# roncapat/UNIGE-TASI-path-planners

Hardware: AMD Instinct MI355X
Metric: grid cells updated/sec (full plan + 100 replans), 4096^2 map (higher is better)
Workload: dtype f32

## Files before the change

unige-tasi-path-planners_amd/csrc/ufm_control.h:

```cpp
#pragma once

__global__ void k_fill(float *p, size_t n, float v) {
    for (size_t i = (size_t)blockIdx.x * blockDim.x + threadIdx.x; i < n; i += (size_t)gridDim.x * blockDim.x) p[i] = v;
}

__device__ __forceinline__ void patch_apply(const DevParams &P, int m, const uint8_t *patch, uint8_t *pmask, int x, int y, int w, int h, int e) {
    if (e >= w * h) return;
    const int i = e / w, j = e - i * w;
    uint8_t *cm = P.cost + (size_t)m * P.cstride;
    const size_t ci = (size_t)(x + i) * P.W + (y + j);
    const uint8_t nv = patch[e];
    const uint8_t ch = cm[ci] != nv;
    pmask[e] = ch;
    if (ch) { cm[ci] = nv; cost_window_store(P, m, x + i, y + j, nv); }
}
__global__ void k_patch_apply(DevParams P, int m, const uint8_t *patch, uint8_t *pmask, int x, int y, int w, int h) {
    patch_apply(P, m, patch, pmask, x, y, w, h, blockIdx.x * blockDim.x + threadIdx.x);
}
template <bool NODES>
__device__ __forceinline__ void patch_seed(const DevParams &P, int m, const uint8_t *pmask, int x, int y, int w, int h, int e) {
    const int ew = NODES ? w + 1 : w, eh = NODES ? h + 1 : h;
    bool hit = false;
    int gt = -1;
    if (e < ew * eh) {
// ... 305 lines not shown
            else if (ug - ur > 8) ++n_low;
            else {
                const int miss = dep_dfm(ga, gp, th) & ~(b & 3);
                auto moved = [&](float v) { return v == INFINITY || abs(__float_as_int(v) - ur) > 8; };
                if (((miss & 1) && moved(q_dfm(INFINITY, gp, th))) || ((miss & 2) && moved(q_dfm(ga, INFINITY, th)))) {
                    if (below_key()) ++n_dep; else ++n_parked;
                }
            }
            continue;
        }
        const int cx = x - 1 + (q >> 1), cy = y - 1 + (q & 1);
        const float c = cst(cx, cy), g1 = h ? val(x, y + dy) : val(x + dx, y), g2 = val(x + dx, y + dy);
        float r; int dep;
        if constexpr (ALGO == UFM_ALGO_SG) { CellSG k; k.set(c); r = tri_sg(g1, g2, k); dep = dep_sg(g1, g2, k); }
        else {
            const float bb = h ? cst(x - 1 + (1 - (q >> 1)), cy) : cst(cx, y - 1 + (1 - (q & 1)));
            CellFD k{c, c * c, c * SQRT2F}; TriFD t; t.set(c, bb);
            r = tri_fd(g1, g2, k, t); dep = dep_fd(g1, g2, k, t);
        }
        if (r > g || r != r) {
            const float B = P.dyn->focused ? start_bound(P, m) : INFINITY;
            if (g + tile_heuristic(P, m, x / T, y / T) < B || B == INFINITY) ++n_bad; else ++n_parked;
        }
        else if (r < g) ++n_low;
        else if (dep != (b & 3)) ++n_dep;
    }
    if (n_val) atomicAdd(&out[0], n_val);
    if (n_none) atomicAdd(&out[1], n_none);
    if (n_bad) atomicAdd(&out[2], n_bad);
    if (n_dep) atomicAdd(&out[3], n_dep);
    if (n_low) atomicAdd(&out[4], n_low);
    if (n_parked) atomicAdd(&out[5], n_parked);
}
__global__ void k_cost_stats(const uint8_t *cm, size_t n, int thr, unsigned long long *out) {
    unsigned long long s = 0, c = 0;
    for (size_t i = (size_t)blockIdx.x * blockDim.x + threadIdx.x; i < n; i += (size_t)gridDim.x * blockDim.x) {
        const int v = cm[i];
        if (v < thr) { s += v; ++c; }
    }
    for (int o = 32; o > 0; o >>= 1) { s += __shfl_down(s, o); c += __shfl_down(c, o); }
    if ((threadIdx.x & 63) == 0) { atomicAdd(&out[0], s); atomicAdd(&out[1], c); }
}
__device__ __forceinline__ void finalize_tiles(const DevParams &P) {
    const int n = P.ctr->tcount;
    for (int i = blockIdx.x; i < n; i += gridDim.x) {
        const int gt = P.tlist[i];
        const size_t gidx = (size_t)gt * TT + threadIdx.x;
        const int diff = (threadIdx.x < T * T) && (P.fresh[gt] ? (P.G[gidx] != INFINITY) : (P.G[gidx] != P.Gprev[gidx]));
        const int c = __syncthreads_count(diff);
        if (threadIdx.x == 0) {
            if (c) atomicAdd(&P.ctr->expanded, (unsigned long long)c);
            P.touched[gt] = 0;
        }
    }
}
__global__ __launch_bounds__(256) void k_finalize(DevParams P, int only_if_done) {
    if (only_if_done && !P.ctr->done) return;
    const int n = P.ctr->tcount;
    const int lane = threadIdx.x & 63;
    const int wave = (blockIdx.x * blockDim.x + threadIdx.x) >> 6, nwaves = (gridDim.x * blockDim.x) >> 6;
    unsigned long long total = 0;
    for (int i = wave; i < n; i += nwaves) {
        const int gt = P.tlist[i];
        const float *g = P.G + (size_t)gt * TT, *g0 = P.Gprev + (size_t)gt * TT;
        int c = 0;
        if (P.fresh[gt]) {
#pragma unroll
            for (int e = lane; e < TT; e += 64) c += (g[e] != INFINITY) ? 1 : 0;
        } else {
#pragma unroll
            for (int e = lane; e < TT; e += 64) c += (g[e] != g0[e]) ? 1 : 0;
        }
        total += (unsigned long long)c;
        if (lane == 0) P.touched[gt] = 0;
    }
    for (int o = 32; o > 0; o >>= 1) total += __shfl_down(total, o);
    if (lane == 0 && total) atomicAdd(&P.ctr->expanded, total);
}
template <int ALGO>
__device__ void tile_bp(const DevParams &P, int gt, int thr, float *Gs, float *Cs) {
    constexpr int CROWS = is_dfm<ALGO> ? T : T + 1, COFF = is_dfm<ALGO> ? 0 : 1, CN = CROWS * CROWS;
    const int tid = threadIdx.x, w = tid >> 6, lane = tid & 63, q = lane & 3, nd = lane >> 2;
    const int m = gt / P.NTm, t = gt - m * P.NTm, tx = t / P.TY, ty = t - tx * P.TY, x0 = tx * T, y0 = ty * T;
    const float *Gt = P.G + (size_t)gt * TT, *ring = P.ring + (size_t)gt * RING;
    const uint8_t *ct = P.costT + (size_t)gt * CTS;
    for (int e = tid; e < TT; e += 256) Gs[(e / T + 1) * GP + e % T + 1] = Gt[e];
    for (int ht = tid; ht < 4 * T + 4; ht += 256) {
        int hr, hc;
        if (ht < T) { hr = -1; hc = ht; }
        else if (ht < 2 * T) { hr = T; hc = ht - T; }
        else if (ht < 3 * T) { hr = ht - 2 * T; hc = -1; }
        else if (ht < 4 * T) { hr = ht - 3 * T; hc = T; }
        else { hr = (ht & 2) ? T : -1; hc = (ht & 1) ? T : -1; }
        Gs[(hr + 1) * GP + hc + 1] = ring[ht];
    }
    for (int e = tid; e < CN; e += 256) {
        const int cr = e / CROWS, cc = e - cr * CROWS, cx = x0 + cr - COFF, cy = y0 + cc - COFF, c = ct[e];
        Cs[cr * CP + cc] = (cx < 0 || cy < 0 || cx >= P.L || cy >= P.W || c >= thr) ? INFINITY : (float)c;
    }
    __syncthreads();
    const int goal_x = P.goal[2 * m], goal_y = P.goal[2 * m + 1];
    for (int p = w; p < PT * PT; p += 4) {
        const int lx = (p / PT) * 4 + (nd >> 2), ly = (p % PT) * 4 + (nd & 3);
        QuadConsts<ALGO> C;
        C.load(Cs, lx, ly, q);
        const LaneEval le = eval_quad_w<ALGO>(Gs + (lx + 1) * GP + ly + 1, q, C);
        const float nv = quad_min(le.r);
        const int bq = quad_min_int(bp_byte<ALGO>(le, q, C, le.r == nv)), b = bp_of_key<ALGO>(bq);
        if (q == 0) P.bp[(size_t)gt * TT + lx * T + ly] = (uint8_t)((x0 + lx == goal_x && y0 + ly == goal_y) ? BP_NONE : b);
    }
    __syncthreads();
}
template <int ALGO>
__global__ __launch_bounds__(256) void k_finalize_bp(DevParams P, int only_if_done) {
    __shared__ float Gs[(T + 2) * GP];
    __shared__ float Cs[(T + 1) * CP];
    if (only_if_done && !P.ctr->done) return;
    const int n = P.ctr->tcount, thr = P.dyn->thr;
    for (int i = blockIdx.x; i < n; i += gridDim.x) tile_bp<ALGO>(P, P.tlist[i], thr, Gs, Cs);
}
__global__ __launch_bounds__(T * T) void k_replan_end(DevParams P, int kr, int kl, float margin,
                                                      DevCounters *host, unsigned int *flag, unsigned int seq) {
    __shared__ int s_m, s_done, s_last;
    kr = launch_index(P, Q_RAISE, kr);
    kl = launch_index(P, Q_LOWER, kl);
    if (seq == 0) seq = P.ctr->pubseq;
    const int done = replan_check(P, kr, kl, margin, blockIdx.x == 0, s_m, s_done);
    if (done) finalize_tiles(P);
    __threadfence();
    __syncthreads();
    if (threadIdx.x == 0) s_last = (atomicAdd(&P.ctr->fin_blocks, 1) == (int)gridDim.x - 1);
    __syncthreads();
    if (!s_last) return;
    __threadfence();
    if (threadIdx.x == 0) P.ctr->fin_blocks = 0;
    const int *src = reinterpret_cast<const int *>(P.ctr);
    int *dst = reinterpret_cast<int *>(host);
    for (int i = threadIdx.x; i < (int)(sizeof(DevCounters) / sizeof(int)); i += blockDim.x)
        dst[i] = __hip_atomic_load(&src[i], __ATOMIC_RELAXED, __HIP_MEMORY_SCOPE_AGENT);
    __threadfence_system();
    __syncthreads();
    if (threadIdx.x == 0) __hip_atomic_store(flag, seq, __ATOMIC_RELEASE, __HIP_MEMORY_SCOPE_SYSTEM);
}
struct ReplanBegin { StepBegin sb; int nrect; int rect[4][5]; int k_raise; float band; };
__device__ void replan_begin(const DevParams &P, const ReplanBegin &a, int &s_keep) {
    step_begin(P, a.sb);
    for (int r = 0; r < a.nrect; ++r) {
        const int *q = a.rect[r];
        for (int e = threadIdx.x; e < (q[3] + 1) * (q[4] + 1); e += blockDim.x) clear_mark(P, q[0], q[1], q[2], q[3], q[4], e);
    }
    __syncthreads();
    seeds_to_active(P, Q_RAISE, a.k_raise, s_keep);
// ... 31 lines not shown
```

unige-tasi-path-planners_amd/csrc/ufm_engine.hip:

```cpp
#include <hip/hip_runtime.h>
#include <hip/hip_ext.h>

#include <algorithm>
#include <chrono>
#include <climits>
#include <cmath>
#include <cstddef>
#include <cstdint>
#include <cstdio>
#include <cstdlib>
#include <cstring>
#include <memory>
#include <new>
#include <type_traits>
#include <thread>
#include <vector>

#include "../../include/ufm.h"

namespace {

#include "ufm_defs.h"
#include "ufm_ops.h"
#include "ufm_relax.h"
#include "ufm_control.h"

#include "ufm_region.h"
#include "ufm_cspace.h"
#include "ufm_census.h"
#include "ufm_sensor.h"
#include "ufm_prepare.h"
#include "ufm_layers.h"

#include "ufm_host.h"
#include "ufm_map_host.h"
#include "ufm_delta.h"

}

struct ufm_planner { Engine *e; };
struct ufm_batch { std::vector<Engine *> shards; int n_maps = 0, per = 1; };

extern "C" {

#ifdef UFM_SWEEPSTAT
int ufm_debug_sstat(unsigned long long *out, int reset) {
    if (out && hipMemcpyFromSymbol(out, HIP_SYMBOL(g_sstat), sizeof(unsigned long long) * 32) != hipSuccess) return UFM_ERR_HIP_BASE;
    if (reset) { unsigned long long z[32] = {}; if (hipMemcpyToSymbol(HIP_SYMBOL(g_sstat), z, sizeof(z)) != hipSuccess) return UFM_ERR_HIP_BASE; }
    return UFM_OK;
}
#endif
#ifdef UFM_TIMING
int ufm_debug_trace(unsigned long long *out, int cap) {
    unsigned int n = 0;
    if (hipMemcpyFromSymbol(&n, HIP_SYMBOL(g_ntrace), sizeof(n)) != hipSuccess) return UFM_ERR_HIP_BASE;
    if ((int)n > cap) n = cap;
    if (n > 16384) n = 16384;
    if (n && hipMemcpyFromSymbol(out, HIP_SYMBOL(g_trace), sizeof(unsigned long long) * 4 * n) != hipSuccess) return UFM_ERR_HIP_BASE;
    const unsigned int z = 0;
    hipMemcpyToSymbol(HIP_SYMBOL(g_ntrace), &z, sizeof(z));
// ... 503 lines not shown
```

unige-tasi-path-planners_amd/csrc/ufm_host.h:

```cpp
#pragma once

#define HIPCHK(expr)                                                      \
    do {                                                                  \
        hipError_t _e = (expr);                                           \
        if (_e != hipSuccess) return UFM_ERR_HIP_BASE - (int)_e;          \
    } while (0)

#include "ufm_route.h"
#include "ufm_patch_route.h"
#include "ufm_path.h"

static_assert(RJOBS <= ROUTE_MAX_JOBS && RTMAX >= 3, "ufm_route.h places at most ROUTE_MAX_JOBS blocks");
constexpr RouteConfig ROUTE_CONFIG{T, RTMAX, RJOBS, ROUTE_MAX_RECTS, 65 * 65};

template <int V> using IntC = std::integral_constant<int, V>;
template <class F> void with_lower_op(int algo, F &&f) {
    if (algo == UFM_ALGO_FD) f(IntC<UFM_ALGO_FD>{});
    else if (algo == UFM_ALGO_SG) f(IntC<UFM_ALGO_SG>{});
    else f(IntC<ALGO_DFM1>{});
}
template <class F> void with_raise_op(int algo, bool follow_info, F &&f) {
    if (algo == UFM_ALGO_DFM && follow_info) f(IntC<ALGO_DFM1_INFO>{});
    else with_lower_op(algo, f);
}
// ... 58 lines not shown
    bool fuse_control = true;
    bool use_graph = true;
    bool use_owned = true;
    float owned_limit_ms = -1.0f;
    float owned_band = -1.0f;
    uint32_t owned_launches = 0;
    EventSet<2> own_ev;
    EventSet<2> reg_ev;
    bool own_timed = false;
    int owned_flags = 0;
    int owned_waves = 0;
    bool dfm_follow_info = false;
    bool use_region = true;
    int region_ahead = 2;
    int region_tiles = 6;
    int region_sweeps = 4096;
    int region_debug = 0;
    float region_band = 1.5f;
    uint32_t region_runs = 0, region_done = 0;
    uint32_t region_cont = 0, region_cont_done = 0;
    int cont_raise = 4, cont_lower = 8;
    int batch_margin = 1;
    float raise_margin = 0.25f;
    PinArray<ReplanJob> h_job;
    struct GraphSig { DevParams P; float band, delta; int max_iters, grid, follow; };
    GraphSig graph_sig{};
    std::vector<std::pair<int, hipGraphExec_t>> graphs;
    void relax(int mode, bool dyn, dim3 g, int k_arg, float delta, float rbound, hipEvent_t e0 = nullptr, hipEvent_t e1 = nullptr);
    float band_delta(float scale) const { return delta_abs >= 0.0f ? delta_abs : scale * T * mean_cost; }
    void finalize_bp(int only_if_done) {
        if (algo == UFM_ALGO_DFM && opt_lvl < 1) return;
        with_lower_op(algo, [&](auto a) { k_finalize_bp<a()><<<2048, 256, 0, stream>>>(P, only_if_done); });
    }
    int tail_grid = 96;
    int replan_graph(int nr, int nl, float band, hipGraphExec_t *out);
    void drop_graphs() { for (auto &g : graphs) hipGraphExecDestroy(g.second); graphs.clear(); }
    struct StepScratch {
        PinArray<unsigned long long> acc;
        int *consume = nullptr, *init = nullptr, *init_tiles = nullptr;
        int *goals = nullptr;
        unsigned int *num_updated = nullptr;
        int *start_el = nullptr;
        float *start_pos = nullptr;
        int carve(int n) {
            { int rc = acc.alloc(2 + 6 * (size_t)n); if (rc != UFM_OK) return rc; }
            consume = reinterpret_cast<int *>(acc + 2); init = consume + n; init_tiles = init + n; goals = init_tiles + n;
            num_updated = reinterpret_cast<unsigned int *>(goals + 2 * n); start_el = goals + 3 * n;
            start_pos = reinterpret_cast<float *>(start_el + 4 * n);
            return UFM_OK;
        }
    } scratch;
    int *d_scratch = nullptr;
    GrowArray<float> d_field;
    GrowArray<int32_t> d_info;
    GrowArray<PathJob> d_jobs;
    GrowArray<float> d_path;
    std::vector<MapState> maps;
    std::vector<PatchRect> pending;
    int iter[2] = {0, 0};
    bool focused = true;
    bool start_cell_floor = false;
    bool dynamic_mode = true;
    PinArray<float> h_bnd;
    int last_active = 1;
    int grid_relax = 512;
    int dyn_grid = 256;
    int small_grid = 1 << 30;
    int max_iters = 32;
    float delta_abs = -1.0f;
    float delta_scale = 1.5f;
    float delta_scale_long = 2.0f;
    float mean_cost = 1.0f;
    int batch_fixed = 0;
    bool profiling = false;
    EventSet<4> chain_ev;
    std::vector<EventSet<1>> batch_ev;
    int batch_ev_slot = 64;
    hipEvent_t batch_event(int slot, int i) const { return batch_ev[(size_t)slot * batch_ev_slot + i][0]; }
    ufm_stats last{};

    std::vector<DevRow> buffer_rows();
    int alloc(int width, int length);
    void release();
    void launch_relax(int mode, float rbound, hipEvent_t e0 = nullptr, hipEvent_t e1 = nullptr);
    int fetch_counters();
    int wait_published();
    int wait_flag(const unsigned int *flag, unsigned int seq);
    int win_raise[6] = {8, 8, 8, 8, 8, 8}, win_lower[6] = {8, 8, 8, 8, 8, 8}, win_pos = 0;
    int run_phase(int mode, float rbound, uint32_t *launches, float *kernel_ms, uint32_t *timed);
    int owned_phase();
    void own_layout(int ys) {
        P.own_ys = ys; P.own_nw = 16 << ys;
        P.own_sx = (P.TX + 15) / 16; P.own_sy = (P.TY + (1 << ys) - 1) >> ys;
        P.own_slots = nmaps * P.own_sx * P.own_sy;
    }
    size_t own_words() const {
        const size_t sx = (size_t)(P.TX + 15) / 16;
        return (size_t)nmaps * sx * std::max<size_t>(256 * (size_t)((P.TY + 15) / 16), 512 * (size_t)((P.TY + 31) / 32));
    }
    int profile_stride = 4;
    int reset_queues();
    int read_bounds(float *bmax);
    struct StepRun {
        StepPlan plan;
        ufm_stats st;
// ... 718 lines not shown
        uint32_t ll = 0;
        k_unpark<<<1, 1024, 0, stream>>>(P, Q_LOWER, iter[Q_LOWER], INFINITY);
        int owned_left = -1;
        if (use_owned && pl.n_init > 0 && round == 0 && dyn_grid >= 256) {
            int rc = owned_phase();
            if (rc != UFM_OK) return rc;
            st.launches += 1u;
            st.resident_launches += 1u;
            rc = fetch_counters();
            if (rc != UFM_OK) return rc;
            owned_left = h_ctr->cnt[Q_LOWER][iter[Q_LOWER] % 3];
        }
        int rc = owned_left == 0 ? UFM_OK : run_phase(MODE_LOWER, INFINITY, &ll, &st.kernel_ms, &st.timed_launches);
        if (rc != UFM_OK) return rc;
        st.launches += ll;
        bool again = false;
        if (focused && do_raise) {
            float bnew = 0.0f;
            rc = read_bounds(&bnew);
            if (rc != UFM_OK) return rc;
            k_queue_min<<<1, 1024, 0, stream>>>(P, Q_RAISE, iter[Q_RAISE]);
            rc = fetch_counters();
            if (rc != UFM_OK) return rc;
            float qm;
            std::memcpy(&qm, &h_ctr->qmin[Q_RAISE], sizeof(float));
            if (qm < bnew) { again = true; rbound = std::fmax(bnew, rbound) + r.band; }
        }
        const auto tc = std::chrono::steady_clock::now();
        r.u_acc += std::chrono::duration<double, std::milli>(tb - ta).count();
        r.p_acc += std::chrono::duration<double, std::milli>(tc - tb).count();
        if (!again) break;
    }
    const auto td = std::chrono::steady_clock::now();
    finalize_bp(0);
    k_finalize<<<2048, 256, 0, stream>>>(P, 0);
    { int rc = fetch_counters(); if (rc != UFM_OK) return rc; }
    copy_counters(st);
    if (st.resident_launches) {
        st.resident_tile_visits = h_ctr->own_vis1 - h_ctr->own_vis0;
        st.resident_stops = (uint32_t)h_ctr->own_stops;
        if (own_timed) HIPCHK(hipEventElapsedTime(&st.resident_kernel_ms, own_ev[0], own_ev[1]));
    }
    if (profiling) {
        std::vector<int> lm(LMAX);
        HIPCHK(hipMemcpy(lm.data(), P.lmax, sizeof(int) * LMAX, hipMemcpyDeviceToHost));
        for (int v : lm) st.crit_sweeps += (uint64_t)v;
    }
    r.p_acc += std::chrono::duration<double, std::milli>(std::chrono::steady_clock::now() - td).count();
    return UFM_OK;
}

void Engine::copy_counters(ufm_stats &st) const {
    st.expanded = h_ctr->expanded;
    st.tile_visits = h_ctr->tile_visits;
    st.tile_iters = h_ctr->tile_iters;
    st.elem_evals = h_ctr->elem_evals;
    st.raise_tile_visits = h_ctr->raise_visits;
}

int Engine::step(ufm_stats *out, const float *auto_mult) {
    for (int m = 0; m < nmaps; ++m) if (!maps[m].have_map) return UFM_LOOP_FAILURE_NO_GRAPH;
    for (int m = 0; m < nmaps; ++m) if (!maps[m].goal_set) return UFM_LOOP_FAILURE_NO_GOAL;
    StepRun r{};
    r.t0 = std::chrono::steady_clock::now();
    r.nr = r.nl = 1;
    for (int i = 0; i < 6; ++i) { r.nr = std::max(r.nr, win_raise[i] + batch_margin); r.nl = std::max(r.nl, win_lower[i] + batch_margin); }
    r.plan = plan_step(ROUTE_CONFIG, route_switches(), maps.data(), pending.data(), (int)pending.size(), (int)lazy.size(), r.nr, r.nl,
                       scratch.consume, scratch.init);
    const StepPlan &pl = r.plan;
    float mult = heuristic_multiplier;
    if (auto_multiplier && heur) {
        if (auto_mult) mult = *auto_mult;
        else { int mn = 0, mx = 0; const int rc = census_minmax(&mn, &mx); if (rc != UFM_OK) return rc; mult = (float)mn; }
    }
    last_multiplier = mult;
    r.dyn_now = DevDyn{heur ? mult : 0.0f, thr_uchar, focused ? 1 : 0, 0};
    r.dyn_pending = std::memcmp(&r.dyn_now, &dyn_dev, sizeof(DevDyn)) != 0;
    r.band = raise_margin * band_delta(delta_scale);
    { int rc = begin_step(r); if (rc != UFM_OK) return rc; }
    r.t_seed = std::chrono::steady_clock::now();
    if (pl.route == Route::SeedsOnly) { int rc = seed_only(r); if (rc != UFM_OK) return rc; }
    else if (pl.route != Route::None) { int rc = replan(r); if (rc != UFM_OK) return rc; }
    if (r.n_init_tiles > 0) {
        HIPCHK(hipMemcpyAsync(d_scratch, scratch.init_tiles, sizeof(int) * r.n_init_tiles, hipMemcpyHostToDevice, stream));
        k_activate_list<<<1, 64, 0, stream>>>(P, Q_LOWER, iter[Q_LOWER], d_scratch, r.n_init_tiles);
    }
    const bool do_plan = (pl.n_init > 0 || r.updated > 0 || (pl.have_seeds && pl.n_upd > 0)) && !r.fast_done;
    r.u_acc = std::chrono::duration<double, std::milli>(std::chrono::steady_clock::now() - r.t0).count();
    if (do_plan) {
        int rc = converge(r);
        if (rc != UFM_OK) return rc;
    } else if (r.fast_done) {
        copy_counters(r.st);
        const double dt = std::chrono::duration<double, std::milli>(std::chrono::steady_clock::now() - r.t_seed).count();
        r.u_acc += 0.5 * dt;
        r.p_acc += 0.5 * dt;
    } else {
        HIPCHK(hipStreamSynchronize(stream));
    }
    for (int m = 0; m < nmaps; ++m) maps[m].new_goal = maps[m].initialize_search = false;
    ufm_stats &st = r.st;
    st.updated = r.updated;
    st.queued_lower = (uint32_t)(h_ctr->cnt[Q_LOWER][iter[Q_LOWER] % 3] + h_ctr->npark[Q_LOWER]);
    st.queued_raise = (uint32_t)(h_ctr->cnt[Q_RAISE][iter[Q_RAISE] % 3] + h_ctr->npark[Q_RAISE]);
    st.graphs_instantiated = graphs_made;
    st.region_replans = region_runs; st.region_replans_done = region_done;
    reveal_busy = false;
    st.u_ms = (float)r.u_acc;
    st.p_ms = (float)r.p_acc;
    last = st;
    if (out) *out = st;
    return UFM_OK;
}

int engine_create(Engine **out, int n_maps, int algo, int opt_lvl, int use_heuristic, int device_id) {
    if (!out || n_maps < 1 || algo < 0 || algo > 2 || opt_lvl < 0 || opt_lvl > 2) return UFM_ERR_INVALID;
    if (algo != UFM_ALGO_SG && opt_lvl > 1) return UFM_ERR_INVALID;
    int ndev = 0;
    HIPCHK(hipGetDeviceCount(&ndev));
    if (device_id < 0 || device_id >= ndev) return UFM_ERR_INVALID;
    HIPCHK(hipSetDevice(device_id));
    std::unique_ptr<Engine> e(new (std::nothrow) Engine());
    if (!e) return UFM_ERR_NOMEM;
    e->algo = algo; e->opt_lvl = opt_lvl; e->heur = use_heuristic; e->device = device_id; e->nmaps = n_maps;
    if (algo == UFM_ALGO_DFM && n_maps == 1) { e->delta_scale = e->delta_scale_long = 2.5f; e->max_iters = 16; }
    if (algo == UFM_ALGO_DFM) { e->cont_lower = 0; e->region_tiles = 8; e->region_ahead = 3; }
    e->maps.resize(n_maps);
    hipDeviceProp_t prop;
    HIPCHK(hipGetDeviceProperties(&prop, device_id));
    e->grid_relax = prop.multiProcessorCount * 2;
    e->dyn_grid = prop.multiProcessorCount;
    HIPCHK(hipStreamCreateWithFlags(&e->stream.s, hipStreamNonBlocking));
    for (Published<DevCounters> *pub : {&e->h_ctr, &e->h_pipe_ctr[0], &e->h_pipe_ctr[1]}) { int rc = pub->alloc(); if (rc != UFM_OK) return rc; }
    { int rc = e->h_job.alloc(1, Pin::Coherent); if (rc != UFM_OK) return rc; }
    std::memset(e->h_job, 0, sizeof(ReplanJob));
    {
        hipGraph_t g = nullptr;
        hipGraphExec_t ge = nullptr;
        if (hipStreamBeginCapture(e->stream, hipStreamCaptureModeThreadLocal) == hipSuccess) {
            k_fill<<<1, 64, 0, e->stream>>>(reinterpret_cast<float *>(e->h_job.p), 0, 0.0f);
            if (hipStreamEndCapture(e->stream, &g) == hipSuccess && g) {
                if (hipGraphInstantiate(&ge, g, nullptr, nullptr, 0) == hipSuccess && ge) {
                    (void)hipGraphLaunch(ge, e->stream);
                    (void)hipStreamSynchronize(e->stream);
                    (void)hipGraphExecDestroy(ge);
                }
                (void)hipGraphDestroy(g);
            }
        }
        (void)hipGetLastError();
    }
    { int rc = e->scratch.carve(n_maps); if (rc != UFM_OK) return rc; }
    { int rc = e->h_bnd.alloc(n_maps); if (rc != UFM_OK) return rc; }
    *out = e.release();
    return UFM_OK;
}

int engine_destroy(Engine *e) {
    if (!e) return UFM_ERR_INVALID;
    delete e;
    return UFM_OK;
}

int engine_set_goal(Engine *e, int m, float x, float y) {
    if (!e || m < 0 || m >= e->nmaps) return UFM_ERR_INVALID;
    MapState &ms = e->maps[m];
    const int ex = (int)std::roundf(x), ey = (int)std::roundf(y);
    ms.new_goal = !ms.goal_set ? true : (ex != ms.goal_ex || ey != ms.goal_ey);
// ... 167 lines not shown
```

unige-tasi-path-planners_amd/csrc/ufm_map_host.h:

```cpp
#pragma once

constexpr PatchRouteConfig PATCH_ROUTE_CONFIG{PATCH_MULTI, 4096, 64, Engine::LAZY_SLOTS};

int Engine::flush_deferred() {
    { int rc = flush_lazy(); if (rc != UFM_OK) return rc; }
    return flush_deferred_only();
}
int Engine::flush_deferred_only() {
    if (deferred.empty()) return UFM_OK;
    PatchMulti a{};
    a.n = (int)deferred.size();
    for (int i = 0; i < a.n; ++i) {
        const DeferredPatch &d = deferred[i];
        put_rect(a.rect[i], PatchRect{d.m, d.x, d.y, d.w, d.h});
        a.ptr[i] = d.ptr;
    }
    deferred.clear();
    with_elements(algo, [&](auto nodes) { k_patch_multi<nodes()><<<a.n, 1024, 0, stream>>>(P, a, d_pmask.dev); });
    HIPCHK(hipGetLastError());
    return UFM_OK;
}
int Engine::ensure_pmask(size_t need) {
    if (need <= d_pmask.cap) return UFM_OK;
    { int rc = flush_deferred_only(); if (rc != UFM_OK) return rc; }
// ... 292 lines not shown
        for (int k = 0; k < n_layers; ++k) j.survey[k] = d_lsurvey[k];
        j.cstride = P.cstride; j.lstride = lstride; j.slot_stride = stride;
        j.n = n_layers; j.nmaps = nmaps; j.L = L; j.W = W; j.mh = sensor.mh; j.mw = sensor.mw; j.ar = sensor.ar; j.ac = sensor.ac;
        hipEvent_t e0, e1;
        { int rc = layer_events(&e0, &e1); if (rc != UFM_OK) return rc; }
        launch(k_reveal_layers, grid, block, stream, e0, e1, j);
    } else {
        RevealJob j{};
        j.mask = d_sensor; j.survey = d_lsurvey[0]; j.cur = cs.on ? d_raw : P.cost; j.slots = d_reveal.dev; j.count = d_reveal_cnt; j.centres = h_centres;
        j.cstride = P.cstride; j.slot_stride = stride;
        j.L = L; j.W = W; j.mh = sensor.mh; j.mw = sensor.mw; j.ar = sensor.ar; j.ac = sensor.ac;
        launch(k_reveal, grid, block, stream, nullptr, nullptr, j);
    }
    HIPCHK(hipGetLastError());
    reveal_busy = true;
    for (int m = first; m < nmaps; ++m) {
        if (centres[2 * m] < 0) continue;
        const int rc = route_patch(PatchSource::RevealSlot, false, 0, d_reveal.dev + stride * (size_t)m, slot_rect(m));
        if (rc != UFM_OK) return rc;
    }
    return UFM_OK;
}
int Engine::reveal_counts(const int32_t *centres, uint64_t *changed) {
    std::vector<unsigned int> cnt((size_t)nmaps, 0u);
    bool any = false;
    for (int m = 0; m < nmaps; ++m) any = any || centres[2 * m] >= 0;
    if (any) HIPCHK(hipMemcpyAsync(cnt.data(), d_reveal_cnt, sizeof(unsigned int) * nmaps, hipMemcpyDeviceToHost, stream));
    HIPCHK(hipStreamSynchronize(stream));
    reveal_busy = false;
    for (int m = 0; m < nmaps; ++m) changed[m] = centres[2 * m] >= 0 ? cnt[m] : 0u;
    return UFM_OK;
}

template <class Fill> int engine_new_raster(Engine *e, int m, int width, int length, Fill &&fill) {
    HIPCHK(hipSetDevice(e->device));
    if (e->allocated) { int rc = e->flush_deferred(); if (rc != UFM_OK) return rc; }
    if (!e->allocated || width != e->W || length != e->L) {
        bool others = false;
        for (int k = 0; k < e->nmaps; ++k) if (k != m && e->maps[k].have_map) others = true;
        if (e->allocated && others) return UFM_ERR_INVALID;
        int rc = e->alloc(width, length);
        if (rc != UFM_OK) return rc;
        if (e->census_on) HIPCHK(hipMemsetAsync(e->d_census, 0, sizeof(uint32_t) * CENSUS_BINS * e->nmaps, e->stream));
    }
    { int rc = fill((e->cs.on ? e->d_raw : e->P.cost) + (size_t)m * e->P.cstride); if (rc != UFM_OK) return rc; }
    if (e->n_layers > 1) {
        HIPCHK(hipMemcpyAsync(e->layer_ptr(0, m), (e->cs.on ? e->d_raw : e->P.cost) + (size_t)m * e->P.cstride, e->P.cstride, hipMemcpyDeviceToDevice, e->stream));
        for (int k = 1; k < e->n_layers; ++k) HIPCHK(hipMemsetAsync(e->layer_ptr(k, m), 0, e->P.cstride, e->stream));
    }
    if (e->cs.on) e->cspace_dilate(m, e->P.cost + (size_t)m * e->P.cstride, width, PatchRect{m, 0, 0, width, length});
    if (e->census_on) { e->census_build(m); e->census_publish(); }
    k_cost_windows<<<2048, 256, 0, e->stream>>>(e->P, m);
    {
        unsigned long long *d_acc = reinterpret_cast<unsigned long long *>(e->d_scratch);
        HIPCHK(hipMemsetAsync(d_acc, 0, 2 * sizeof(unsigned long long), e->stream));
        k_cost_stats<<<512, 256, 0, e->stream>>>(e->P.cost + (size_t)m * e->P.cstride, (size_t)width * length, e->thr_uchar, d_acc);
        unsigned long long *h_acc = e->scratch.acc;
        HIPCHK(hipMemcpyAsync(h_acc, d_acc, 2 * sizeof(unsigned long long), hipMemcpyDeviceToHost, e->stream));
        HIPCHK(hipStreamSynchronize(e->stream));
        if (h_acc[1] > 0) e->mean_cost = (float)((double)h_acc[0] / (double)h_acc[1]);
    }
    if (e->track) { int rc = e->track_reset(m); if (rc != UFM_OK) return rc; }
    e->maps[m].have_map = true;
    MapState &ms = e->maps[m];
    if (ms.goal_set) ms.goal_elem_valid = ms.goal_ex >= 0 && ms.goal_ey >= 0 && ms.goal_ex < e->P.EX && ms.goal_ey < e->P.EY;
    return UFM_OK;
}

int engine_set_map(Engine *e, int m, const uint8_t *src, bool on_device, int width, int length) {
    if (!e || !src || m < 0 || m >= e->nmaps || width <= 0 || length <= 0) return UFM_ERR_INVALID;
    return engine_new_raster(e, m, width, length, [&](uint8_t *dst) -> int {
        HIPCHK(hipMemcpyAsync(dst, src, (size_t)width * length, on_device ? hipMemcpyDeviceToDevice : hipMemcpyHostToDevice, e->stream));
        return UFM_OK;
    });
}

int engine_set_image(Engine *e, int m, const uint8_t *src, bool on_device, int width, int length, const uint16_t *taps, int ntaps, int penalty) {
    PrepTaps k;
    if (!e || !src || m < 0 || m >= e->nmaps || !prep_args_valid(taps, ntaps, width, length, penalty) || !prep_pack(taps, ntaps, &k)) return UFM_ERR_INVALID;
    if (e->allocated && (width != e->W || length != e->L))
        for (int j = 0; j < e->nmaps; ++j) if (j != m && e->maps[j].have_map) return UFM_ERR_INVALID;
    bool timed = false;
    const int rc = engine_new_raster(e, m, width, length, [&](uint8_t *dst) -> int {
        const size_t n = (size_t)width * length, all = e->P.cstride * e->nmaps;
        { int rc2 = e->survey_alloc(0); if (rc2 != UFM_OK) return rc2; }
        uint8_t *survey = e->d_lsurvey[0];
        const uint8_t *image = src;
        if (!on_device || prep_overlap(src, n, e->P.cost, all) || prep_overlap(src, n, survey, all) || (e->cs.on && prep_overlap(src, n, e->d_raw, all))) {
            { int rc2 = e->d_image.reserve(e->stream, n); if (rc2 != UFM_OK) return rc2; }
            HIPCHK(hipMemcpyAsync(e->d_image.dev, src, n, on_device ? hipMemcpyDeviceToDevice : hipMemcpyHostToDevice, e->stream));
            image = e->d_image.dev;
        }
        PrepareJob j{};
        j.src = image; j.out_l = dst; j.out_h = survey + (size_t)m * e->P.cstride;
        j.W = width; j.L = length; j.penalty = penalty;
        j.wide_in = width % 4 == 0 && prep_aligned4(j.src);
        j.wide_out = width % 4 == 0 && prep_aligned4(j.out_l) && prep_aligned4(j.out_h);
        j.taps = k;
        timed = e->profiling;
        if (timed) { int rc2 = e->prep_ev.ensure(); if (rc2 != UFM_OK) return rc2; }
        launch(k_prepare, dim3(prep_grid_x(width), prep_grid_y(length)), dim3(PREP_THREADS), e->stream, timed ? e->prep_ev[0] : nullptr,
               timed ? e->prep_ev[1] : nullptr, j);
        HIPCHK(hipGetLastError());
        e->have_lsurvey[0][m] = 1;
        return UFM_OK;
    });
    if (rc != UFM_OK) return rc;
    e->reveal_busy = false;
    if (timed) HIPCHK(hipEventElapsedTime(&e->prep_ms, e->prep_ev[0], e->prep_ev[1]));
    return UFM_OK;
}

int engine_read_map(Engine *e, int m, uint8_t *host_map) {
    if (!e || !host_map || !e->allocated || m < 0 || m >= e->nmaps) return UFM_ERR_INVALID;
    HIPCHK(hipSetDevice(e->device));
    { int rc = e->flush_deferred(); if (rc != UFM_OK) return rc; }
// ... 12 lines not shown
```

unige-tasi-path-planners_amd/csrc/ufm_ops.h:

```cpp
#pragma once

#ifdef UFM_SWEEPSTAT
__device__ unsigned long long g_sstat[32];
#endif
__device__ __forceinline__ float sqrt_rn(float x) {
    float s = __builtin_amdgcn_sqrtf(x);
    const float sm = __int_as_float(__float_as_int(s) - 1);
    const float sp = __int_as_float(__float_as_int(s) + 1);
    const float rm = __builtin_fmaf(-sm, s, x);
    const float rp = __builtin_fmaf(-sp, s, x);
    s = (rm <= 0.0f) ? sm : s;
    s = (rp > 0.0f) ? sp : s;
    return s;
}

struct CellSG {
    float cadd;
    float ccmp;
    float c2, cs2;
    __device__ __forceinline__ void set(float c) {
        cadd = c; ccmp = (c == INFINITY) ? -1.0f : c; c2 = c * c; cs2 = c * SQRT2F;
    }
};
__device__ __forceinline__ float tri_sg(float g1, float g2, const CellSG &K) {
// ... 176 lines not shown
}
template <int ALGO, int GPITCH = GP>
__device__ __forceinline__ float eval_quad(const float *ctr, int q, const QuadConsts<ALGO> &C) {
    if constexpr (ALGO == ALGO_DFM1) {
        const float pm = fminf(ctr[-C.po], ctr[C.po]);
        return fminf(q_dfm(ctr[-C.so], pm, C.th), q_dfm(ctr[C.so], pm, C.th));
    } else {
        const int sx = (q & 2) ? GPITCH : -GPITCH, sy = (q & 1) ? 1 : -1;
        const float gD = ctr[sx + sy], gV = ctr[sx], gH = ctr[sy];
        if constexpr (ALGO == UFM_ALGO_SG)
            return fminf(tri_sg(gV, gD, C.k), tri_sg(gH, gD, C.k));
        else
            return fminf(tri_fd(gV, gD, C.k, C.tv), tri_fd(gH, gD, C.k, C.th));
    }
}

__device__ __forceinline__ void cost_window_store(const DevParams &P, int m, int cx, int cy, uint8_t v) {
    const int bx = cx / T, by = cy / T, rx = cx % T, ry = cy % T;
    if (P.cells) {
        P.costT[((size_t)m * P.NTm + (size_t)bx * P.TY + by) * CTS + rx * T + ry] = v;
        return;
    }
#pragma unroll
    for (int dx = 0; dx < 2; ++dx)
#pragma unroll
        for (int dy = 0; dy < 2; ++dy) {
            if ((dx && rx != T - 1) || (dy && ry != T - 1)) continue;
            const int tx = bx + dx, ty = by + dy;
            if (tx >= P.TX || ty >= P.TY) continue;
            const int cr = dx ? 0 : rx + 1, cc = dy ? 0 : ry + 1;
            P.costT[((size_t)m * P.NTm + (size_t)tx * P.TY + ty) * CTS + cr * (T + 1) + cc] = v;
        }
}
__global__ void k_cost_windows(DevParams P, int m) {
    const int crows = P.cells ? T : T + 1, off = P.cells ? 0 : 1, per = crows * crows;
    const uint8_t *cm = P.cost + (size_t)m * P.cstride;
    const size_t n = (size_t)P.NTm * per;
    for (size_t i = (size_t)blockIdx.x * blockDim.x + threadIdx.x; i < n; i += (size_t)gridDim.x * blockDim.x) {
        const int t = (int)(i / per), e = (int)(i - (size_t)t * per);
        const int tx = t / P.TY, ty = t - tx * P.TY, cr = e / crows, cc = e - cr * crows;
        const int cx = tx * T + cr - off, cy = ty * T + cc - off;
        const bool in = cx >= 0 && cy >= 0 && cx < P.L && cy < P.W;
        P.costT[((size_t)m * P.NTm + t) * CTS + e] = in ? cm[(size_t)cx * P.W + cy] : (uint8_t)255;
    }
}
```

Measured before the change: 598.9 million.

## Fuse cost window build with cost stats and defer mean-cost sync; fuse finalize count into bp

Replaces the separate cost-window kernel and cost-stats reduction with one tile-per-wave kernel. It reads each map row with wide loads, writes the tile window through LDS, and accumulates the mean-cost sums in the same pass. The host synchronize after map upload is deferred until the mean cost is actually needed at the next step, using a flag published by the last block. Full-plan finalization now counts changed cells inside the backpointer kernel instead of launching a second finalize kernel. The cost is more complex last-block reduction and flag logic, plus a risk of stale mean_cost ordering.

```diff
diff --git a/unige-tasi-path-planners_amd/csrc/ufm_control.h b/unige-tasi-path-planners_amd/csrc/ufm_control.h
--- a/unige-tasi-path-planners_amd/csrc/ufm_control.h
+++ b/unige-tasi-path-planners_amd/csrc/ufm_control.h
@@ -361,15 +361,6 @@
     if (n_low) atomicAdd(&out[4], n_low);
     if (n_parked) atomicAdd(&out[5], n_parked);
 }
-__global__ void k_cost_stats(const uint8_t *cm, size_t n, int thr, unsigned long long *out) {
-    unsigned long long s = 0, c = 0;
-    for (size_t i = (size_t)blockIdx.x * blockDim.x + threadIdx.x; i < n; i += (size_t)gridDim.x * blockDim.x) {
-        const int v = cm[i];
-        if (v < thr) { s += v; ++c; }
-    }
-    for (int o = 32; o > 0; o >>= 1) { s += __shfl_down(s, o); c += __shfl_down(c, o); }
-    if ((threadIdx.x & 63) == 0) { atomicAdd(&out[0], s); atomicAdd(&out[1], c); }
-}
 __device__ __forceinline__ void finalize_tiles(const DevParams &P) {
     const int n = P.ctr->tcount;
     for (int i = blockIdx.x; i < n; i += gridDim.x) {
@@ -406,13 +397,22 @@
     for (int o = 32; o > 0; o >>= 1) total += __shfl_down(total, o);
     if (lane == 0 && total) atomicAdd(&P.ctr->expanded, total);
 }
-template <int ALGO>
-__device__ void tile_bp(const DevParams &P, int gt, int thr, float *Gs, float *Cs) {
+template <int ALGO, bool COUNT = false>
+__device__ int tile_bp(const DevParams &P, int gt, int thr, float *Gs, float *Cs) {
     constexpr int CROWS = is_dfm<ALGO> ? T : T + 1, COFF = is_dfm<ALGO> ? 0 : 1, CN = CROWS * CROWS;
     const int tid = threadIdx.x, w = tid >> 6, lane = tid & 63, q = lane & 3, nd = lane >> 2;
     const int m = gt / P.NTm, t = gt - m * P.NTm, tx = t / P.TY, ty = t - tx * P.TY, x0 = tx * T, y0 = ty * T;
     const float *Gt = P.G + (size_t)gt * TT, *ring = P.ring + (size_t)gt * RING;
     const uint8_t *ct = P.costT + (size_t)gt * CTS;
+    int changed = 0;
+    if constexpr (COUNT) {
+        const float *G0 = P.fresh[gt] ? nullptr : P.Gprev + (size_t)gt * TT;
+        for (int e = tid; e < TT; e += 256) {
+            const float g = Gt[e];
+            Gs[(e / T + 1) * GP + e % T + 1] = g;
+            changed += (G0 ? g != G0[e] : g != INFINITY) ? 1 : 0;
+        }
+    } else
     for (int e = tid; e < TT; e += 256) Gs[(e / T + 1) * GP + e % T + 1] = Gt[e];
     for (int ht = tid; ht < 4 * T + 4; ht += 256) {
         int hr, hc;
@@ -439,6 +439,7 @@
         if (q == 0) P.bp[(size_t)gt * TT + lx * T + ly] = (uint8_t)((x0 + lx == goal_x && y0 + ly == goal_y) ? BP_NONE : b);
     }
     __syncthreads();
+    return changed;
 }
 template <int ALGO>
 __global__ __launch_bounds__(256) void k_finalize_bp(DevParams P, int only_if_done) {
@@ -447,6 +448,26 @@
     if (only_if_done && !P.ctr->done) return;
     const int n = P.ctr->tcount, thr = P.dyn->thr;
     for (int i = blockIdx.x; i < n; i += gridDim.x) tile_bp<ALGO>(P, P.tlist[i], thr, Gs, Cs);
+}
+template <int ALGO>
+__global__ __launch_bounds__(256) void k_finalize_count_bp(DevParams P) {
+    __shared__ float Gs[(T + 2) * GP];
+    __shared__ float Cs[(T + 1) * CP];
+    __shared__ unsigned long long s_cnt[4];
+    const int n = P.ctr->tcount, thr = P.dyn->thr;
+    unsigned long long total = 0;
+    for (int i = blockIdx.x; i < n; i += gridDim.x) {
+        const int gt = P.tlist[i];
+        total += (unsigned long long)tile_bp<ALGO, true>(P, gt, thr, Gs, Cs);
+        if (threadIdx.x == 0) P.touched[gt] = 0;
+    }
+    for (int o = 32; o > 0; o >>= 1) total += __shfl_down(total, o);
+    if ((threadIdx.x & 63) == 0) s_cnt[threadIdx.x >> 6] = total;
+    __syncthreads();
+    if (threadIdx.x == 0) {
+        const unsigned long long c = s_cnt[0] + s_cnt[1] + s_cnt[2] + s_cnt[3];
+        if (c) atomicAdd(&P.ctr->expanded, c);
+    }
 }
 __global__ __launch_bounds__(T * T) void k_replan_end(DevParams P, int kr, int kl, float margin,
                                                       DevCounters *host, unsigned int *flag, unsigned int seq) {
diff --git a/unige-tasi-path-planners_amd/csrc/ufm_cost_pass.h b/unige-tasi-path-planners_amd/csrc/ufm_cost_pass.h
--- /dev/null
+++ b/unige-tasi-path-planners_amd/csrc/ufm_cost_pass.h
@@ -0,0 +1,96 @@
+#pragma once
+
+struct CostPassJob {
+    const uint8_t *cm;
+    uint8_t *costT;
+    unsigned long long *acc;
+    unsigned long long *out;
+    unsigned int *flag;
+    unsigned int seq;
+    int L, W, TX, TY;
+    int cells;
+    int thr;
+    int wide;
+};
+constexpr int COST_PASS_THREADS = 256, COST_PASS_WAVES = COST_PASS_THREADS / 64, COST_PASS_GRID = 2048, COST_PASS_ACC = 1 + 2 * COST_PASS_GRID;
+inline int cost_pass_grid(int tiles) { return std::max(1, std::min(COST_PASS_GRID, (tiles + COST_PASS_WAVES - 1) / COST_PASS_WAVES)); }
+
+__global__ __launch_bounds__(COST_PASS_THREADS) void k_cost_pass(CostPassJob J) {
+    __shared__ uint32_t s_win[COST_PASS_WAVES][CTS / 4];
+    __shared__ unsigned long long s_red[2 * COST_PASS_WAVES];
+    __shared__ int s_last;
+    const int lane = threadIdx.x & 63, w = threadIdx.x >> 6;
+    const int rows = J.cells ? T : T + 1, off = J.cells ? 0 : 1, per = rows * rows;
+    const int NT = J.TX * J.TY;
+    uint8_t *win = reinterpret_cast<uint8_t *>(s_win[w]);
+    unsigned int ls = 0, lc = 0;
+    for (int t = (int)blockIdx.x * COST_PASS_WAVES + w; t < NT; t += (int)gridDim.x * COST_PASS_WAVES) {
+        if (lane < rows) {
+            const int tx = t / J.TY, ty = t - tx * J.TY;
+            const int cx = tx * T + lane - off, cy0 = ty * T;
+            const bool row_in = cx >= 0 && cx < J.L, own = lane >= off;
+            const uint8_t *src = J.cm + (size_t)(row_in ? cx : 0) * J.W;
+            uint8_t *dst = win + lane * rows;
+            if (off) dst[0] = (row_in && cy0 >= 1 && cy0 - 1 < J.W) ? src[cy0 - 1] : (uint8_t)255;
+            dst += off;
+            if (J.wide && row_in && cy0 + T <= J.W) {
+#pragma unroll
+                for (int k = 0; k < T / 16; ++k) {
+                    const uint4 v = *reinterpret_cast<const uint4 *>(src + cy0 + 16 * k);
+                    const uint32_t q[4] = {v.x, v.y, v.z, v.w};
+#pragma unroll
+                    for (int j = 0; j < 16; ++j) {
+                        const int b = (int)((q[j >> 2] >> (8 * (j & 3))) & 255u);
+                        dst[16 * k + j] = (uint8_t)b;
+                        if (own && b < J.thr) { ls += (unsigned int)b; ++lc; }
+                    }
+                }
+            } else {
+                for (int j = 0; j < T; ++j) {
+                    const bool in = row_in && cy0 + j < J.W;
+                    const int b = in ? (int)src[cy0 + j] : 255;
+                    dst[j] = (uint8_t)b;
+                    if (in && own && b < J.thr) { ls += (unsigned int)b; ++lc; }
+                }
+            }
+        }
+        __builtin_amdgcn_fence(__ATOMIC_RELEASE, "workgroup");
+        __builtin_amdgcn_wave_barrier();
+        __builtin_amdgcn_fence(__ATOMIC_ACQUIRE, "workgroup");
+        uint8_t *rec = J.costT + (size_t)t * CTS;
+        for (int i = lane; i < per / 4; i += 64) reinterpret_cast<uint32_t *>(rec)[i] = s_win[w][i];
+        if (lane < (per & 3)) rec[(per & ~3) + lane] = win[(per & ~3) + lane];
+        __builtin_amdgcn_fence(__ATOMIC_RELEASE, "workgroup");
+        __builtin_amdgcn_wave_barrier();
+    }
+    unsigned long long s = ls, c = lc;
+    for (int o = 32; o > 0; o >>= 1) { s += __shfl_down(s, o); c += __shfl_down(c, o); }
+    if (lane == 0) { s_red[2 * w] = s; s_red[2 * w + 1] = c; }
+    __syncthreads();
+    if (threadIdx.x == 0) {
+        s = c = 0;
+        for (int i = 0; i < COST_PASS_WAVES; ++i) { s += s_red[2 * i]; c += s_red[2 * i + 1]; }
+        J.acc[1 + 2 * blockIdx.x] = s; J.acc[2 + 2 * blockIdx.x] = c;
+        __threadfence();
+        s_last = atomicAdd(&J.acc[0], 1ull) == (unsigned long long)gridDim.x - 1ull;
+    }
+    __syncthreads();
+    if (!s_last) return;
+    __threadfence();
+    s = c = 0;
+    for (int i = threadIdx.x; i < (int)gridDim.x; i += COST_PASS_THREADS) {
+        s += __hip_atomic_load(&J.acc[1 + 2 * i], __ATOMIC_RELAXED, __HIP_MEMORY_SCOPE_AGENT);
+        c += __hip_atomic_load(&J.acc[2 + 2 * i], __ATOMIC_RELAXED, __HIP_MEMORY_SCOPE_AGENT);
+    }
+    for (int o = 32; o > 0; o >>= 1) { s += __shfl_down(s, o); c += __shfl_down(c, o); }
+    __syncthreads();
+    if (lane == 0) { s_red[2 * w] = s; s_red[2 * w + 1] = c; }
+    __syncthreads();
+    if (threadIdx.x != 0) return;
+    s = c = 0;
+    for (int i = 0; i < COST_PASS_WAVES; ++i) { s += s_red[2 * i]; c += s_red[2 * i + 1]; }
+    J.acc[0] = 0;
+    J.out[0] = s; J.out[1] = c;
+    __threadfence_system();
+    __hip_atomic_store(J.flag, J.seq, __ATOMIC_RELEASE, __HIP_MEMORY_SCOPE_SYSTEM);
+}
diff --git a/unige-tasi-path-planners_amd/csrc/ufm_engine.hip b/unige-tasi-path-planners_amd/csrc/ufm_engine.hip
--- a/unige-tasi-path-planners_amd/csrc/ufm_engine.hip
+++ b/unige-tasi-path-planners_amd/csrc/ufm_engine.hip
@@ -26,6 +26,7 @@
 #include "ufm_control.h"
 
 #include "ufm_region.h"
+#include "ufm_cost_pass.h"
 #include "ufm_cspace.h"
 #include "ufm_census.h"
 #include "ufm_sensor.h"
diff --git a/unige-tasi-path-planners_amd/csrc/ufm_host.h b/unige-tasi-path-planners_amd/csrc/ufm_host.h
--- a/unige-tasi-path-planners_amd/csrc/ufm_host.h
+++ b/unige-tasi-path-planners_amd/csrc/ufm_host.h
@@ -114,6 +114,10 @@
         if (algo == UFM_ALGO_DFM && opt_lvl < 1) return;
         with_lower_op(algo, [&](auto a) { k_finalize_bp<a()><<<2048, 256, 0, stream>>>(P, only_if_done); });
     }
+    void finalize_plan() {
+        if (algo == UFM_ALGO_DFM && opt_lvl < 1) k_finalize<<<2048, 256, 0, stream>>>(P, 0);
+        else with_lower_op(algo, [&](auto a) { k_finalize_count_bp<a()><<<2048, 256, 0, stream>>>(P); });
+    }
     int tail_grid = 96;
     int replan_graph(int nr, int nl, float band, hipGraphExec_t *out);
     void drop_graphs() { for (auto &g : graphs) hipGraphExecDestroy(g.second); graphs.clear(); }
@@ -153,6 +157,12 @@
     float delta_scale = 1.5f;
     float delta_scale_long = 2.0f;
     float mean_cost = 1.0f;
+    struct CostSums { unsigned long long sum, count; };
+    Published<CostSums> h_cost;
+    DevArray<unsigned long long> d_cost_acc;
+    unsigned int cost_seq = 0;
+    bool cost_pending = false;
+    int take_mean_cost();
     int batch_fixed = 0;
     bool profiling = false;
     EventSet<4> chain_ev;
@@ -937,8 +947,7 @@
         if (!again) break;
     }
     const auto td = std::chrono::steady_clock::now();
-    finalize_bp(0);
-    k_finalize<<<2048, 256, 0, stream>>>(P, 0);
+    finalize_plan();
     { int rc = fetch_counters(); if (rc != UFM_OK) return rc; }
     copy_counters(st);
     if (st.resident_launches) {
@@ -981,8 +990,9 @@
     last_multiplier = mult;
     r.dyn_now = DevDyn{heur ? mult : 0.0f, thr_uchar, focused ? 1 : 0, 0};
     r.dyn_pending = std::memcmp(&r.dyn_now, &dyn_dev, sizeof(DevDyn)) != 0;
+    { int rc = begin_step(r); if (rc != UFM_OK) return rc; }
+    { int rc = take_mean_cost(); if (rc != UFM_OK) return rc; }
     r.band = raise_margin * band_delta(delta_scale);
-    { int rc = begin_step(r); if (rc != UFM_OK) return rc; }
     r.t_seed = std::chrono::steady_clock::now();
     if (pl.route == Route::SeedsOnly) { int rc = seed_only(r); if (rc != UFM_OK) return rc; }
     else if (pl.route != Route::None) { int rc = replan(r); if (rc != UFM_OK) return rc; }
@@ -1039,6 +1049,9 @@
     for (Published<DevCounters> *pub : {&e->h_ctr, &e->h_pipe_ctr[0], &e->h_pipe_ctr[1]}) { int rc = pub->alloc(); if (rc != UFM_OK) return rc; }
     { int rc = e->h_job.alloc(1, Pin::Coherent); if (rc != UFM_OK) return rc; }
     std::memset(e->h_job, 0, sizeof(ReplanJob));
+    { int rc = e->h_cost.alloc(); if (rc != UFM_OK) return rc; }
+    { int rc = e->d_cost_acc.alloc(COST_PASS_ACC); if (rc != UFM_OK) return rc; }
+    HIPCHK(hipMemsetAsync(e->d_cost_acc, 0, COST_PASS_ACC * sizeof(unsigned long long), e->stream));
     {
         hipGraph_t g = nullptr;
         hipGraphExec_t ge = nullptr;
diff --git a/unige-tasi-path-planners_amd/csrc/ufm_map_host.h b/unige-tasi-path-planners_amd/csrc/ufm_map_host.h
--- a/unige-tasi-path-planners_amd/csrc/ufm_map_host.h
+++ b/unige-tasi-path-planners_amd/csrc/ufm_map_host.h
@@ -348,8 +348,17 @@
     return UFM_OK;
 }
 
-template <class Fill> int engine_new_raster(Engine *e, int m, int width, int length, Fill &&fill) {
-    HIPCHK(hipSetDevice(e->device));
+int Engine::take_mean_cost() {
+    if (!cost_pending) return UFM_OK;
+    if (spin_wait) { int rc = wait_flag(h_cost.flag(), cost_seq); if (rc != UFM_OK) return rc; }
+    else HIPCHK(hipStreamSynchronize(stream));
+    cost_pending = false;
+    if (h_cost->count > 0) mean_cost = (float)((double)h_cost->sum / (double)h_cost->count);
+    return UFM_OK;
+}
+template <class Fill> int engine_new_raster(Engine *e, int m, int width, int length, bool stream_ordered, Fill &&fill) {
+    HIPCHK(hipSetDevice(e->device));
+    { int rc = e->take_mean_cost(); if (rc != UFM_OK) return rc; }
     if (e->allocated) { int rc = e->flush_deferred(); if (rc != UFM_OK) return rc; }
     if (!e->allocated || width != e->W || length != e->L) {
         bool others = false;
@@ -366,15 +375,20 @@
     }
     if (e->cs.on) e->cspace_dilate(m, e->P.cost + (size_t)m * e->P.cstride, width, PatchRect{m, 0, 0, width, length});
     if (e->census_on) { e->census_build(m); e->census_publish(); }
-    k_cost_windows<<<2048, 256, 0, e->stream>>>(e->P, m);
     {
-        unsigned long long *d_acc = reinterpret_cast<unsigned long long *>(e->d_scratch);
-        HIPCHK(hipMemsetAsync(d_acc, 0, 2 * sizeof(unsigned long long), e->stream));
-        k_cost_stats<<<512, 256, 0, e->stream>>>(e->P.cost + (size_t)m * e->P.cstride, (size_t)width * length, e->thr_uchar, d_acc);
-        unsigned long long *h_acc = e->scratch.acc;
-        HIPCHK(hipMemcpyAsync(h_acc, d_acc, 2 * sizeof(unsigned long long), hipMemcpyDeviceToHost, e->stream));
-        HIPCHK(hipStreamSynchronize(e->stream));
-        if (h_acc[1] > 0) e->mean_cost = (float)((double)h_acc[0] / (double)h_acc[1]);
+        CostPassJob j{};
+        j.cm = e->P.cost + (size_t)m * e->P.cstride; j.costT = e->P.costT + (size_t)m * e->P.NTm * CTS;
+        j.acc = e->d_cost_acc; j.out = &e->h_cost->sum; j.flag = e->h_cost.flag(); j.seq = ++e->cost_seq;
+        j.L = length; j.W = width; j.TX = e->P.TX; j.TY = e->P.TY; j.cells = e->P.cells; j.thr = e->thr_uchar;
+        j.wide = width % 16 == 0 && reinterpret_cast<uintptr_t>(j.cm) % 16 == 0;
+        k_cost_pass<<<cost_pass_grid(e->P.NTm), COST_PASS_THREADS, 0, e->stream>>>(j);
+        HIPCHK(hipGetLastError());
+        e->cost_pending = true;
+        if (!stream_ordered || e->census_on) {
+            HIPCHK(hipStreamSynchronize(e->stream));
+            int rc = e->take_mean_cost();
+            if (rc != UFM_OK) return rc;
+        }
     }
     if (e->track) { int rc = e->track_reset(m); if (rc != UFM_OK) return rc; }
     e->maps[m].have_map = true;
@@ -385,7 +399,7 @@
 
 int engine_set_map(Engine *e, int m, const uint8_t *src, bool on_device, int width, int length) {
     if (!e || !src || m < 0 || m >= e->nmaps || width <= 0 || length <= 0) return UFM_ERR_INVALID;
-    return engine_new_raster(e, m, width, length, [&](uint8_t *dst) -> int {
+    return engine_new_raster(e, m, width, length, on_device, [&](uint8_t *dst) -> int {
         HIPCHK(hipMemcpyAsync(dst, src, (size_t)width * length, on_device ? hipMemcpyDeviceToDevice : hipMemcpyHostToDevice, e->stream));
         return UFM_OK;
     });
@@ -397,7 +411,7 @@
     if (e->allocated && (width != e->W || length != e->L))
         for (int j = 0; j < e->nmaps; ++j) if (j != m && e->maps[j].have_map) return UFM_ERR_INVALID;
     bool timed = false;
-    const int rc = engine_new_raster(e, m, width, length, [&](uint8_t *dst) -> int {
+    const int rc = engine_new_raster(e, m, width, length, false, [&](uint8_t *dst) -> int {
         const size_t n = (size_t)width * length, all = e->P.cstride * e->nmaps;
         { int rc2 = e->survey_alloc(0); if (rc2 != UFM_OK) return rc2; }
         uint8_t *survey = e->d_lsurvey[0];
diff --git a/unige-tasi-path-planners_amd/csrc/ufm_ops.h b/unige-tasi-path-planners_amd/csrc/ufm_ops.h
--- a/unige-tasi-path-planners_amd/csrc/ufm_ops.h
+++ b/unige-tasi-path-planners_amd/csrc/ufm_ops.h
@@ -232,15 +232,3 @@
             P.costT[((size_t)m * P.NTm + (size_t)tx * P.TY + ty) * CTS + cr * (T + 1) + cc] = v;
         }
 }
-__global__ void k_cost_windows(DevParams P, int m) {
-    const int crows = P.cells ? T : T + 1, off = P.cells ? 0 : 1, per = crows * crows;
-    const uint8_t *cm = P.cost + (size_t)m * P.cstride;
-    const size_t n = (size_t)P.NTm * per;
-    for (size_t i = (size_t)blockIdx.x * blockDim.x + threadIdx.x; i < n; i += (size_t)gridDim.x * blockDim.x) {
-        const int t = (int)(i / per), e = (int)(i - (size_t)t * per);
-        const int tx = t / P.TY, ty = t - tx * P.TY, cr = e / crows, cc = e - cr * crows;
-        const int cx = tx * T + cr - off, cy = ty * T + cc - off;
-        const bool in = cx >= 0 && cy >= 0 && cx < P.L && cy < P.W;
-        P.costT[((size_t)m * P.NTm + t) * CTS + e] = in ? cm[(size_t)cx * P.W + cy] : (uint8_t)255;
-    }
-}
```

Result: no change. 604.6 million (median of 6 runs) (+1.0%).
